# lukehollis/three-mlagents

Hardware: NVIDIA B200
Metric: env_steps_per_sec (higher is better)
Workload: dtype f32+f64

## Files before the change

### profiles/rollout_ab.py

```python
from __future__ import annotations

import argparse
import json
import os
import shutil
import statistics
import subprocess
import sys
import tempfile

import numpy as np

ROOT = os.path.dirname(os.path.dirname(os.path.abspath(__file__)))


def _run(cmd, cwd):
    r = subprocess.run(cmd, cwd=cwd, capture_output=True, text=True)
    if r.returncode != 0:
        raise RuntimeError(f"{' '.join(cmd)} in {cwd} failed ({r.returncode}):\n{r.stdout[-2000:]}\n{r.stderr[-4000:]}")
    return r.stdout


def _bench(tree, steps, dump=None):
    cmd = [sys.executable, "bench.py", "--quick", "--steps", str(steps)] + (["--dump-outputs", dump] if dump else [])
    return json.loads(_run(cmd, tree).strip().splitlines()[-1])


def main():
    ap = argparse.ArgumentParser()
    ap.add_argument("--parent", required=True, help="untracked export of the parent commit")
    ap.add_argument("--rounds", type=int, default=4)
    ap.add_argument("--steps", type=int, default=200)
    ap.add_argument("--out", default=os.path.join(ROOT, "profiles", "rollout_direct_obs_ab_1gpu.json"))
    args = ap.parse_args()
    trees = {"parent": os.path.abspath(args.parent), "new": ROOT}
    q = "name,power.limit,clocks.max.sm"
    card = _run(["nvidia-smi", f"--query-gpu={q}", "--format=csv,noheader", "-i", "0"], ROOT).strip()
    result = {"card": dict(zip(q.split(","), [c.strip() for c in card.split(",")])),
              "bench": f"bench.py --quick --steps {args.steps}", "rounds": args.rounds}
    for tree in trees.values():
        _run([sys.executable, os.path.join(tree, "three-mlagents_b200", "build.py")], tree)
    tmp = tempfile.mkdtemp(prefix="rollout_ab_")
    try:
        for name, tree in trees.items():
            _bench(tree, 50, dump=os.path.join(tmp, name))
        result["dump_equal"] = {f: bool(np.array_equal(np.load(os.path.join(tmp, "parent", f)), np.load(os.path.join(tmp, "new", f))))
                                for f in ("obs.npy", "actions.npy", "rewards.npy", "dones.npy")}
    finally:
        shutil.rmtree(tmp, ignore_errors=True)
    runs = {name: [] for name in trees}
    for _ in range(args.rounds):
        for name, tree in trees.items():
            runs[name].append(_bench(tree, args.steps)["ms_per_step"] * 1e3)
            print(name, f"{runs[name][-1]:.2f} us", file=sys.stderr, flush=True)
    base = statistics.median(runs["parent"])
    result["runs"] = {name: {"us_per_launch": us, "median_us": statistics.median(us),
                             "spread": (max(us) - min(us)) / statistics.median(us),
                             "gain_vs_parent": 1.0 - statistics.median(us) / base} for name, us in runs.items()}
    os.makedirs(os.path.dirname(os.path.abspath(args.out)), exist_ok=True)
    with open(args.out, "w") as f:
        json.dump(result, f, indent=1)
    print(json.dumps(result))


if __name__ == "__main__":
    main()
```

### three-mlagents_b200/csrc/env_kernels.cu

```cuda
#include <stdarg.h>
#include <stdlib.h>
#include <string.h>
#include <new>
#include <type_traits>
#if defined(__x86_64__)
#include <immintrin.h>
#endif
#include "envs.cuh"
#include "env_handle.cuh"

static int order_after_device_path(tmla_env *h) {
    if (!h->dev_dirty) return TMLA_OK;
    h->dev_dirty = false;
    cudaStreamCaptureStatus cap = cudaStreamCaptureStatusNone;
    if (cudaStreamIsCapturing(h->dev_stream, &cap) != cudaSuccess || cap != cudaStreamCaptureStatusNone ||
        cudaEventRecord(h->dev_evt, h->dev_stream) != cudaSuccess) {
        cudaGetLastError();
        TMLA_CUDA(cudaDeviceSynchronize());
        return TMLA_OK;
    }
    TMLA_CUDA(cudaStreamWaitEvent(h->own_stream, h->dev_evt, 0));
    return TMLA_OK;
}

struct EnvPtrs { void *buf[4]; };

static constexpr int kBlock = 128;

template <int D, int BLOCK, bool STREAMING>
__device__ __forceinline__ void block_store_obs(const float *s_obs, float *dst, int valid_envs) {
    const int total = valid_envs * D;
    if ((reinterpret_cast<uintptr_t>(dst) & 15u) == 0) {
        const int nvec = total >> 2;
        const float4 *s4 = reinterpret_cast<const float4 *>(s_obs);
        float4 *d4 = reinterpret_cast<float4 *>(dst);
        for (int v = threadIdx.x; v < nvec; v += BLOCK) {
            if (STREAMING) st_stream_f4(d4 + v, s4[v]);
            else d4[v] = s4[v];
        }
        for (int e = (nvec << 2) + threadIdx.x; e < total; e += BLOCK) dst[e] = s_obs[e];
    } else {
        for (int e = threadIdx.x; e < total; e += BLOCK) dst[e] = s_obs[e];
    }
}

template <int D>
__device__ __forceinline__ void thread_store_obs(const float *o, float *dst) {
#pragma unroll
    for (int j = 0; j < D; ++j) dst[j] = o[j];
}

template <class Task>
__global__ void __launch_bounds__(kBlock) reset_kernel(EnvPtrs p, int64_t n, uint64_t seed, uint64_t env_base,
                                                       uint64_t k, uint32_t tag, float *obs) {
    __shared__ __align__(16) float s_obs[kBlock * Task::D];
    const int64_t i0 = (int64_t)blockIdx.x * kBlock, i = i0 + threadIdx.x;
    if (i < n) {
        typename Task::State s;
        Task::reset(s, seed, env_base + (uint64_t)i, k, tag);
        Task::store(p.buf, i, s);
        float o[Task::D];
        Task::observe(s, o);
#pragma unroll
        for (int j = 0; j < Task::D; ++j) s_obs[threadIdx.x * Task::D + j] = o[j];
    }
    __syncthreads();
    if (obs) block_store_obs<Task::D, kBlock, false>(s_obs, obs + i0 * Task::D, (int)min((int64_t)kBlock, n - i0));
}

template <class Task>
__global__ void get_state_kernel(EnvPtrs p, int64_t n, typename Task::Wire *aos) {
    const int64_t i = (int64_t)blockIdx.x * blockDim.x + threadIdx.x;
    if (i < n) aos[i] = Task::to_wire(Task::load(p.buf, i));
}
template <class Task>
__global__ void set_state_kernel(EnvPtrs p, int64_t n, const typename Task::Wire *aos) {
    const int64_t i = (int64_t)blockIdx.x * blockDim.x + threadIdx.x;
    if (i < n) Task::store(p.buf, i, Task::from_wire(aos[i]));
}

template <class Task>
__global__ void __launch_bounds__(kBlock)
step_kernel(EnvPtrs p, int64_t n, uint64_t seed, uint64_t env_base, uint64_t step_index,
            const int32_t *__restrict__ actions, float *__restrict__ obs, float *__restrict__ reward,
            uint8_t *__restrict__ done, uint8_t *__restrict__ truncated, float *__restrict__ terminal_obs,
            float *__restrict__ ep_return, int32_t *__restrict__ ep_length, int32_t *n_done, int *err_flag,
            float *__restrict__ compact, int32_t *__restrict__ host_flags, int host_seq, int act_u8,
            const int32_t *ready, int32_t *dev_ready, int chunk_ctas, EnvPtrs shadow) {
    constexpr int D = Task::D;
    __shared__ __align__(16) float s_obs[kBlock * D];
    __shared__ __align__(16) float s_rew[kBlock];
    __shared__ __align__(16) uint8_t s_flag[2 * kBlock];
    const int64_t i0 = (int64_t)blockIdx.x * kBlock, i = i0 + threadIdx.x;
    if (ready) {
        __shared__ int s_go;
        if (threadIdx.x == 0) {
            const int c = blockIdx.x / chunk_ctas;
            const bool leader = blockIdx.x == (unsigned)(c * chunk_ctas);
            const volatile int32_t *f = leader ? ready + c : dev_ready + c;
            unsigned long long t0, t1;
            asm volatile("mov.u64 %0, %%globaltimer;" : "=l"(t0));
            int v;
            while ((v = *f) != host_seq && v != ~host_seq) {
                asm volatile("mov.u64 %0, %%globaltimer;" : "=l"(t1));
                if (t1 - t0 > 2000000000ull) { v = ~host_seq; break; }
                if (leader) __nanosleep(100);
            }
            if (leader) { __threadfence_system(); *(volatile int32_t *)(dev_ready + c) = v; }
            __threadfence_system();
            s_go = v == host_seq;
        }
        __syncthreads();
        if (!s_go) return;
    }
    const bool wide = (n - i0 >= kBlock) && (((reinterpret_cast<uintptr_t>(reward + i0) | reinterpret_cast<uintptr_t>(done + i0) |
                                               reinterpret_cast<uintptr_t>(truncated + i0)) & 15u) == 0);
    if (i < n) {
        const typename Task::Consts cst = Task::load_consts();
        typename Task::State s = Task::load(p.buf, i);
        if (shadow.buf[0]) Task::store(shadow.buf, i, s);
        int a = act_u8 ? (int)reinterpret_cast<const uint8_t *>(actions)[i] : actions[i];
        if ((unsigned)a >= (unsigned)Task::A) { *err_flag = 1; a = min(max(a, 0), Task::A - 1); }
        float r; bool term, trunc;
        Task::step(cst, s, a, r, term, trunc);
        s.ep_ret = __fadd_rn(s.ep_ret, r);
        const bool d = term || trunc;
        if (wide) {
            s_rew[threadIdx.x] = r;
            s_flag[threadIdx.x] = d ? 1 : 0;
            s_flag[kBlock + threadIdx.x] = (trunc && !term) ? 1 : 0;
        } else {
            reward[i] = r;
            done[i] = d ? 1 : 0;
            truncated[i] = (trunc && !term) ? 1 : 0;
        }
        float o[D];
        Task::observe(s, o);
        if (d) {
            if (terminal_obs) thread_store_obs<D>(o, terminal_obs + i * D);
            if (ep_return) ep_return[i] = s.ep_ret;
            if (ep_length) ep_length[i] = s.steps;
            int slot = 0;
            if (n_done) slot = atomicAdd(n_done, 1);
            if (compact) {
                constexpr int RW = (3 + D + 3) & ~3;
                float rec[RW];
                rec[0] = __int_as_float((int)i); rec[1] = s.ep_ret; rec[2] = __int_as_float(s.steps);
#pragma unroll
                for (int j = 0; j < D; ++j) rec[3 + j] = o[j];
#pragma unroll
                for (int j = 3 + D; j < RW; ++j) rec[j] = 0.0f;
                float4 *dst = reinterpret_cast<float4 *>(compact + (int64_t)slot * RW);
#pragma unroll
                for (int q = 0; q < RW / 4; ++q) dst[q] = make_float4(rec[4 * q], rec[4 * q + 1], rec[4 * q + 2], rec[4 * q + 3]);
            }
            Task::reset(s, seed, env_base + (uint64_t)i, step_index + 1, TMLA_TAG_RESET);
            Task::observe(s, o);
        }
        Task::store(p.buf, i, s);
#pragma unroll
        for (int j = 0; j < D; ++j) s_obs[threadIdx.x * D + j] = o[j];
    }
    __syncthreads();
    block_store_obs<D, kBlock, false>(s_obs, obs + i0 * D, (int)min((int64_t)kBlock, n - i0));
    if (wide) {
        const int t = threadIdx.x;
        if (t < kBlock / 4) reinterpret_cast<float4 *>(reward + i0)[t] = reinterpret_cast<const float4 *>(s_rew)[t];
        else if (t < kBlock / 4 + kBlock / 16) reinterpret_cast<uint4 *>(done + i0)[t - kBlock / 4] = reinterpret_cast<const uint4 *>(s_flag)[t - kBlock / 4];
        else if (t < kBlock / 4 + kBlock / 8) reinterpret_cast<uint4 *>(truncated + i0)[t - kBlock / 4 - kBlock / 16] = reinterpret_cast<const uint4 *>(s_flag + kBlock)[t - kBlock / 4 - kBlock / 16];
    }
    if (host_flags) {
        __syncthreads();
        if (threadIdx.x == 0) {
            __threadfence_system();
            if (atomicAdd(n_done + 2, 1) == (int)gridDim.x - 1) {
                __threadfence();
                host_flags[0] = *(volatile int32_t *)n_done;
                host_flags[1] = *(volatile int32_t *)(n_done + 1);
                n_done[0] = 0; n_done[1] = 0; n_done[2] = 0;
                __threadfence_system();
                *(volatile int32_t *)(host_flags + 2) = host_seq;
            }
        }
    }
}

static constexpr int kRollBlock = 32;

template <int D>
__device__ __forceinline__ void stage_obs(float *stage, const float *o) {
    if (D % 2 == 0) {
        float2 *s2 = reinterpret_cast<float2 *>(stage + threadIdx.x * D);
#pragma unroll
        for (int j = 0; j < D / 2; ++j) s2[j] = make_float2(o[2 * j], o[2 * j + 1]);
    } else {
#pragma unroll
        for (int j = 0; j < D; ++j) stage[threadIdx.x * D + j] = o[j];
    }
}

template <class Task>
__global__ void __launch_bounds__(kRollBlock)
rollout_random_kernel(EnvPtrs p, int64_t n, uint64_t seed, uint64_t env_base, uint64_t step0, int T,
                      float *__restrict__ obs_buf, int32_t *__restrict__ act_buf, float *__restrict__ rew_buf,
                      uint8_t *__restrict__ done_buf) {
    constexpr int D = Task::D, BLOCK = kRollBlock;
    constexpr bool STAGED = (D != 4);
    constexpr int NVEC = BLOCK * D / 4;
    __shared__ __align__(16) float s_obs[STAGED ? 2 * BLOCK * D : 4];
    const int64_t i0 = (int64_t)blockIdx.x * BLOCK, i = i0 + threadIdx.x;
    const bool active = i < n;
    const int valid = (int)min((int64_t)BLOCK, n - i0);
    const uint64_t env_id = env_base + (uint64_t)i;
    const int64_t row_floats = n * D;
    const bool vec_ok = obs_buf && valid == BLOCK && ((reinterpret_cast<uintptr_t>(obs_buf + i0 * D) & 15u) == 0) &&
                        ((row_floats & 3) == 0);
    const typename Task::Consts cst = Task::load_consts();
    typename Task::State s;
    TmlaActionStream as;
    if (active) {
        s = Task::load(p.buf, i);
        as.seek(seed, env_id, step0, Task::A);
    }
    float *orow = obs_buf ? obs_buf + i0 * D : nullptr;
    int64_t off = i;
    for (int t = 0; t < T; ++t) {
        const uint64_t k = step0 + (uint64_t)t;
        float *stage = STAGED ? s_obs + (t & 1) * BLOCK * D : s_obs;
        if (active) {
            float o[D];
            Task::observe(s, o);
            if (STAGED) stage_obs<D>(stage, o);
            else if (obs_buf) {
                float *dst = obs_buf + off * 4;
                if ((reinterpret_cast<uintptr_t>(obs_buf) & 15u) == 0) st_stream_f4(reinterpret_cast<float4 *>(dst), make_float4(o[0], o[1], o[2], o[3]));
                else { dst[0] = o[0]; dst[1] = o[1]; dst[2] = o[2]; dst[3] = o[3]; }
            }
            const int a = as.next(seed, env_id, step0, (uint32_t)t, Task::A);
            float r; bool term, trunc;
            Task::step(cst, s, a, r, term, trunc);
            s.ep_ret = __fadd_rn(s.ep_ret, r);
            const bool d = term || trunc;
            if (act_buf) __stcs(act_buf + off, a);
            if (rew_buf) __stcs(rew_buf + off, r);
            if (done_buf) __stcs(done_buf + off, (uint8_t)(d ? 1 : 0));
            if (d) Task::reset(s, seed, env_id, k + 1, TMLA_TAG_RESET);
        }
        if (STAGED) {
            __syncthreads();
            if (vec_ok) {
                const float4 *s4 = reinterpret_cast<const float4 *>(stage);
                float4 *d4 = reinterpret_cast<float4 *>(orow);
#pragma unroll
                for (int v = 0; v < (NVEC + BLOCK - 1) / BLOCK; ++v) {
                    const int e = v * BLOCK + threadIdx.x;
                    if ((v + 1) * BLOCK <= NVEC || e < NVEC) st_stream_f4(d4 + e, s4[e]);
                }
            } else if (obs_buf) {
                block_store_obs<D, BLOCK, true>(stage, orow, valid);
            }
            if (orow) orow += row_floats;
        }
        off += n;
    }
    if (active) Task::store(p.buf, i, s);
}

#ifndef TMLA_SPARE_EVERY
#define TMLA_SPARE_EVERY 64
#endif
static constexpr int kSpareEvery = TMLA_SPARE_EVERY;
#ifndef TMLA_ROLLOUT_UNROLL
#define TMLA_ROLLOUT_UNROLL 2
#endif
static constexpr int kRollUnroll = TMLA_ROLLOUT_UNROLL;
static_assert((kSpareEvery & (kSpareEvery - 1)) == 0, "power of two");
template <class Task>
__global__ void __launch_bounds__(kRollBlock)
rollout_fast_kernel(EnvPtrs p, uint32_t n, uint64_t seed, uint64_t env_base, uint64_t step0, int T,
                    float4 *__restrict__ obs4, int32_t *__restrict__ act_buf, float *__restrict__ rew_buf,
                    uint8_t *__restrict__ done_buf) {
    constexpr int D = Task::D, BLOCK = kRollBlock, NVEC = BLOCK * D / 4;
    constexpr bool DIRECT = (D == 6);
    constexpr bool STAGED = (D != 4) && !DIRECT;
    static_assert((BLOCK * D) % 4 == 0, "block rows must be whole float4s");
    __shared__ __align__(16) float s_stage[STAGED ? 2 * BLOCK * D : 4];
    const uint32_t tid = threadIdx.x, i = blockIdx.x * BLOCK + tid;
    const uint64_t env_id = env_base + (uint64_t)i;
    const typename Task::Consts cst = Task::load_consts();
    typename Task::State s = Task::load(p.buf, i);
    TmlaActionStream as;
    as.seek(seed, env_id, step0, Task::A);
    uint32_t off = i;
    uint32_t voff = blockIdx.x * NVEC + tid;
    const uint32_t rowvec = n / 4 * D;
    uint32_t sb = 0;
    [[maybe_unused]] typename Task::Spare sp;
    [[maybe_unused]] bool have_spare = false;
#pragma unroll kRollUnroll
    for (int t = 0; t < T; ++t) {
        if constexpr (Task::HAS_SPARE) {
            if ((t & (kSpareEvery - 1)) == 0 && !have_spare) {
                sp = Task::draw(seed, env_id, Task::next_episode(s), TMLA_TAG_RESET);
                have_spare = true;
            }
        }
        float o[D];
        Task::observe(s, o);
        if constexpr (STAGED) {
            if constexpr (D % 2 == 0) {
                float2 *s2 = reinterpret_cast<float2 *>(s_stage + sb + tid * D);
#pragma unroll
                for (int j = 0; j < D / 2; ++j) s2[j] = make_float2(o[2 * j], o[2 * j + 1]);
            } else {
#pragma unroll
                for (int j = 0; j < D; ++j) s_stage[sb + tid * D + j] = o[j];
            }
        } else if constexpr (DIRECT) {
            float2 *d2 = reinterpret_cast<float2 *>(reinterpret_cast<float *>(obs4) + (size_t)off * D);
#pragma unroll
            for (int j = 0; j < D / 2; ++j) __stcs(d2 + j, make_float2(o[2 * j], o[2 * j + 1]));
        } else {
            st_stream_f4(obs4 + off, make_float4(o[0], o[1], o[2], o[3]));
        }
        const int a = as.next(seed, env_id, step0, (uint32_t)t, Task::A);
        float r; bool term, trunc;
        Task::step(cst, s, a, r, term, trunc);
        s.ep_ret = __fadd_rn(s.ep_ret, r);
        const bool d = term || trunc;
        __stcs(act_buf + off, a);
        __stcs(rew_buf + off, r);
        __stcs(done_buf + off, (uint8_t)(d ? 1 : 0));
        if (d) {
            if constexpr (Task::HAS_SPARE) {
                const uint32_t e = Task::next_episode(s);
                if (!have_spare) sp = Task::draw(seed, env_id, e, TMLA_TAG_RESET);
                Task::begin_episode(s, sp, e);
                have_spare = false;
            } else {
                Task::reset(s, seed, env_id, step0 + (uint64_t)t + 1, TMLA_TAG_RESET);
            }
        }
        if constexpr (STAGED) {
            if constexpr (BLOCK == 32) __syncwarp(); else __syncthreads();
            const float4 *s4 = reinterpret_cast<const float4 *>(s_stage + sb);
#pragma unroll
            for (int v = 0; v < (NVEC + BLOCK - 1) / BLOCK; ++v) {
                const int e = v * BLOCK + tid;
                if ((v + 1) * BLOCK <= NVEC || e < NVEC) st_stream_f4(obs4 + voff + v * BLOCK, s4[e]);
            }
            sb ^= BLOCK * D;
            voff += rowvec;
        }
        off += n;
    }
    Task::store(p.buf, i, s);
}

template <int A>
__device__ __forceinline__ void categorical(const float *l, bool deterministic, float u, int &action, float &logp) {
    float m = l[0];
#pragma unroll
    for (int j = 1; j < A; ++j) m = fmaxf(m, l[j]);
    float e[A], sum = 0.0f;
#pragma unroll
    for (int j = 0; j < A; ++j) { e[j] = expf(l[j] - m); sum += e[j]; }
    int a = 0;
    if (deterministic) {
#pragma unroll
        for (int j = 1; j < A; ++j) if (l[j] > l[a]) a = j;
    } else {
        const float target = u * sum;
        float c = 0.0f;
        a = A - 1;
        bool found = false;
#pragma unroll
        for (int j = 0; j < A; ++j) {
            c += e[j];
            if (!found && target < c) { a = j; found = true; }
        }
    }
    action = a;
    logp = (l[a] - m) - logf(sum);
}

template <class Task>
__global__ void __launch_bounds__(kBlock)
step_policy_kernel(EnvPtrs p, int64_t n, uint64_t seed, uint64_t env_base, uint64_t step_index,
                   const uint64_t *__restrict__ step_base, const float *__restrict__ logits, int deterministic,
                   int64_t row_index, float *__restrict__ obs_next, int32_t *__restrict__ act, float *__restrict__ logp_out,
                   float *__restrict__ rew, uint8_t *__restrict__ done, int32_t *trunc_count,
                   int32_t *__restrict__ trunc_index, float *__restrict__ trunc_obs, int32_t trunc_capacity,
                   float *ep_stats, float2 *__restrict__ ep_log, int32_t ep_log_cap, int32_t *ep_log_count) {
    constexpr int D = Task::D, A = Task::A;
    __shared__ __align__(16) float s_obs[kBlock * D];
    __shared__ float s_ep[3];
    const int64_t i0 = (int64_t)blockIdx.x * kBlock, i = i0 + threadIdx.x;
    const uint64_t k = step_base ? (*step_base + (uint64_t)row_index) : step_index;
    const unsigned lane = threadIdx.x & 31u, lanes_below = (1u << lane) - 1u;
    if (threadIdx.x < 3) s_ep[threadIdx.x] = 0.0f;
    __syncthreads();
    const bool live = i < n;
    const uint64_t env_id = env_base + (uint64_t)i;
    typename Task::State s;
    float o[D];
    bool d = false, trunc_only = false;
    float ep_r = 0.0f, ep_l = 0.0f;
    if (live) {
        const typename Task::Consts cst = Task::load_consts();
        s = Task::load(p.buf, i);
        float l[A];
#pragma unroll
        for (int j = 0; j < A; ++j) l[j] = logits[i * A + j];
        float u = 0.0f;
        if (!deterministic) u = tmla_u24(tmla_stream_block(seed, env_id, k, TMLA_TAG_SAMPLE, 0).x);
        int a; float lp;
        categorical<A>(l, deterministic != 0, u, a, lp);
        float r; bool term, trunc;
        Task::step(cst, s, a, r, term, trunc);
        s.ep_ret = __fadd_rn(s.ep_ret, r);
        d = term || trunc;
        trunc_only = trunc && !term;
        if (act) act[i] = a;
        if (logp_out) logp_out[i] = lp;
        rew[i] = r;
        done[i] = d ? 1 : 0;
        Task::observe(s, o);
        if (d) { ep_r = s.ep_ret; ep_l = (float)s.steps; }
    }
    if (trunc_count) {
        const unsigned m = __ballot_sync(0xffffffffu, trunc_only);
        if (m) {
            const int leader = __ffs(m) - 1;
            int base = 0;
            if ((int)lane == leader) base = atomicAdd(trunc_count, __popc(m));
            base = __shfl_sync(0xffffffffu, base, leader);
            if (trunc_only) {
                const int slot = base + __popc(m & lanes_below);
                if (slot < trunc_capacity) {
                    trunc_index[slot] = (int32_t)(row_index * n + i);
                    thread_store_obs<D>(o, trunc_obs + (int64_t)slot * D);
                }
            }
        }
    }
    const unsigned dm = __ballot_sync(0xffffffffu, d);
    if (dm) {
        if (ep_stats) {
            float wr = ep_r, wl = ep_l;
#pragma unroll
            for (int sh = 16; sh > 0; sh >>= 1) { wr += __shfl_xor_sync(0xffffffffu, wr, sh); wl += __shfl_xor_sync(0xffffffffu, wl, sh); }
            if (lane == 0) { atomicAdd(s_ep + 0, wr); atomicAdd(s_ep + 1, wl); atomicAdd(s_ep + 2, (float)__popc(dm)); }
        }
        if (ep_log) {
            const int leader = __ffs(dm) - 1;
            int base = 0;
            if ((int)lane == leader) base = atomicAdd(ep_log_count, __popc(dm));
            base = __shfl_sync(0xffffffffu, base, leader);
            if (d) {
                const int slot = base + __popc(dm & lanes_below);
                if (slot < ep_log_cap) ep_log[slot] = make_float2(ep_r, ep_l);
            }
        }
    }
    if (live) {
        if (d) {
            Task::reset(s, seed, env_id, k + 1, TMLA_TAG_RESET);
            Task::observe(s, o);
        }
        Task::store(p.buf, i, s);
#pragma unroll
        for (int j = 0; j < D; ++j) s_obs[threadIdx.x * D + j] = o[j];
    }
    __syncthreads();
    if (ep_stats && threadIdx.x == 0 && s_ep[2] > 0.0f) {
        atomicAdd(ep_stats + 0, s_ep[0]);
        atomicAdd(ep_stats + 1, s_ep[1]);
        atomicAdd(ep_stats + 2, s_ep[2]);
    }
    block_store_obs<D, kBlock, false>(s_obs, obs_next + i0 * D, (int)min((int64_t)kBlock, n - i0));
}

__global__ void counter_add_kernel(uint64_t *c, uint64_t n) { *c += n; }

__global__ void selftest_arith_kernel(unsigned long long *out) {
    const uint32_t tid = blockIdx.x * blockDim.x + threadIdx.x, nth = gridDim.x * blockDim.x;
    unsigned long long bad3 = 0;
    for (uint32_t bits = tid; bits < 0x41000000u; bits += nth) {
        const float x = __uint_as_float(bits);
        bad3 += (__float_as_uint(div3_rn(x)) != __float_as_uint(__fdiv_rn(x, 3.0f)));
    }
    if (bad3) atomicAdd(out + 0, bad3);
    if (tid < 11) {
        const float k = (float)((int)tid - 5);
        if (__float_as_uint(div5_rn(k)) != __float_as_uint(__fdiv_rn(k, 5.0f))) atomicAdd(out + 1, 1ull);
    }
    unsigned long long worst = 0;
    for (uint32_t j = tid; j < (1u << 22); j += nth) {
        const double x = kB3.max_tilt * (2.0 * ((double)j + 0.5) / 4194304.0 - 1.0);
        const long long a = __double_as_longlong(sin_small(x)), b = __double_as_longlong(sin(x));
        const unsigned long long d = (unsigned long long)(a > b ? a - b : b - a);
        worst = d > worst ? d : worst;
    }
    atomicMax(out + 2, worst);
}

#define TASK_SWITCH(task, CALL)                                   \
    switch (task) {                                               \
        case TMLA_BASIC: { using TaskT = BasicTask; CALL; } break;        \
        case TMLA_BALL3D: { using TaskT = Ball3DTask; CALL; } break;      \
        case TMLA_GRIDWORLD: { using TaskT = GridWorldTask; CALL; } break; \
        case TMLA_PUSH: { using TaskT = PushTask; CALL; } break;          \
        case TMLA_WALLJUMP: { using TaskT = WallJumpTask; CALL; } break;  \
        case TMLA_BRICKBREAK: { using TaskT = BrickBreakTask; CALL; } break; \
        case TMLA_BICYCLE: { using TaskT = BicycleTask; CALL; } break;       \
        case TMLA_GLIDER: { using TaskT = GliderTask; CALL; } break;         \
        default: tmla_set_error("unknown task %d", task); return TMLA_EINVAL; \
    }

static EnvPtrs ptrs_of(const tmla_env *h) {
    EnvPtrs p;
    for (int b = 0; b < 4; ++b) p.buf[b] = h->buf[b];
    return p;
}
static inline unsigned grid_for(int64_t n) { return (unsigned)ceil_div64(n, kBlock); }

static const int kObsDim[TMLA_NUM_TASKS] = {BasicTask::D, Ball3DTask::D, GridWorldTask::D, PushTask::D, WallJumpTask::D, BrickBreakTask::D, BicycleTask::D, GliderTask::D};
static const int kNumActions[TMLA_NUM_TASKS] = {BasicTask::A, Ball3DTask::A, GridWorldTask::A, PushTask::A, WallJumpTask::A, BrickBreakTask::A, BicycleTask::A, GliderTask::A};
static const int kMaxSteps[TMLA_NUM_TASKS] = {BasicTask::MAX_STEPS, Ball3DTask::MAX_STEPS, GridWorldTask::MAX_STEPS, PushTask::MAX_STEPS,
                                              WallJumpTask::MAX_STEPS, BrickBreakTask::MAX_STEPS, BicycleTask::MAX_STEPS, GliderTask::MAX_STEPS};
static const int kStateSize[TMLA_NUM_TASKS] = {(int)sizeof(tmla_basic_state), (int)sizeof(tmla_ball3d_state), (int)sizeof(tmla_gridworld_state),
                                               (int)sizeof(tmla_push_state), (int)sizeof(tmla_walljump_state), (int)sizeof(tmla_brickbreak_state),
                                               (int)sizeof(tmla_bicycle_state), (int)sizeof(tmla_glider_state)};

static inline int record_words(int D) { return (3 + D + 3) & ~3; }
struct StageLayout { size_t act, obs, rew, done, trunc, flags, crec, tobs, ret, len, end; };
static StageLayout stage_layout(int64_t n, int D) {
    auto up = [](size_t x) { return (x + 15) & ~(size_t)15; };
    StageLayout L;
    L.act = 0;
    L.obs = up(L.act + 4 * n);
    L.rew = L.obs + 4 * n * D;
    L.done = L.rew + 4 * n;
    L.trunc = L.done + n;
    L.flags = up(L.trunc + n);
    L.crec = L.flags + 16;
    L.tobs = up(L.crec + 4 * n * record_words(D));
    L.ret = L.tobs + 4 * n * D;
    L.len = L.ret + 4 * n;
    L.end = L.len + 4 * n;
    return L;
}


#if defined(__x86_64__)
__attribute__((target("avx2"))) static int64_t stage_actions32_avx2(const int32_t *src, uint8_t *dst, int64_t n, uint64_t *ored, uint32_t *mx) {
    __m256i acc = _mm256_setzero_si256(), vmx = _mm256_setzero_si256();
    const __m256i perm = _mm256_setr_epi32(0, 4, 1, 5, 2, 6, 3, 7);
    int64_t i = 0;
    for (; i + 32 <= n; i += 32) {
        const __m256i a = _mm256_loadu_si256((const __m256i *)(src + i)), b = _mm256_loadu_si256((const __m256i *)(src + i + 8));
        const __m256i c = _mm256_loadu_si256((const __m256i *)(src + i + 16)), d = _mm256_loadu_si256((const __m256i *)(src + i + 24));
        acc = _mm256_or_si256(acc, _mm256_or_si256(_mm256_or_si256(a, b), _mm256_or_si256(c, d)));
        __m256i p = _mm256_packus_epi16(_mm256_packs_epi32(a, b), _mm256_packs_epi32(c, d));
        p = _mm256_permutevar8x32_epi32(p, perm);
        vmx = _mm256_max_epu8(vmx, p);
        _mm256_storeu_si256((__m256i *)(dst + i), p);
    }
    uint64_t t[4]; uint8_t m8[32];
    _mm256_storeu_si256((__m256i *)t, acc); _mm256_storeu_si256((__m256i *)m8, vmx);
    const uint64_t o = t[0] | t[1] | t[2] | t[3];
    *ored |= (o | (o >> 32)) & 0xFFFFFFFFull;
    for (int k = 0; k < 32; ++k) *mx = m8[k] > *mx ? m8[k] : *mx;
    return i;
}
__attribute__((target("avx2"))) static int64_t stage_actions64_avx2(const int64_t *src, uint8_t *dst, int64_t n, uint64_t *ored, uint32_t *mx) {
    __m256i acc = _mm256_setzero_si256(), vmx = _mm256_setzero_si256();
    const __m256i lo = _mm256_setr_epi32(0, 2, 4, 6, 0, 2, 4, 6), perm = _mm256_setr_epi32(0, 4, 1, 5, 2, 6, 3, 7);
    int64_t i = 0;
    for (; i + 32 <= n; i += 32) {
        __m256i w[4];
        for (int k = 0; k < 4; ++k) {
            const __m256i x = _mm256_loadu_si256((const __m256i *)(src + i + 8 * k)), y = _mm256_loadu_si256((const __m256i *)(src + i + 8 * k + 4));
            acc = _mm256_or_si256(acc, _mm256_or_si256(x, y));
            const __m256i xl = _mm256_permutevar8x32_epi32(x, lo), yl = _mm256_permutevar8x32_epi32(y, lo);
            w[k] = _mm256_inserti128_si256(xl, _mm256_castsi256_si128(yl), 1);
        }
        __m256i p = _mm256_packus_epi16(_mm256_packs_epi32(w[0], w[1]), _mm256_packs_epi32(w[2], w[3]));
        p = _mm256_permutevar8x32_epi32(p, perm);
        vmx = _mm256_max_epu8(vmx, p);
        _mm256_storeu_si256((__m256i *)(dst + i), p);
    }
    uint64_t t[4]; uint8_t m8[32];
    _mm256_storeu_si256((__m256i *)t, acc); _mm256_storeu_si256((__m256i *)m8, vmx);
    const uint64_t o = t[0] | t[1] | t[2] | t[3];
    *ored |= (o & ~7ull) ? 0xFFFFFFFFull : (o & 7ull);
    for (int k = 0; k < 32; ++k) *mx = m8[k] > *mx ? m8[k] : *mx;
    return i;
}
#endif

extern "C" {

int tmla_task_from_name(const char *name) {
    if (!name) { tmla_set_error("task name is NULL"); return TMLA_EINVAL; }
    if (!strcmp(name, "basic")) return TMLA_BASIC;
    if (!strcmp(name, "ball3d")) return TMLA_BALL3D;
    if (!strcmp(name, "gridworld")) return TMLA_GRIDWORLD;
    if (!strcmp(name, "push")) return TMLA_PUSH;
    if (!strcmp(name, "walljump")) return TMLA_WALLJUMP;
    if (!strcmp(name, "brickbreak")) return TMLA_BRICKBREAK;
    if (!strcmp(name, "bicycle")) return TMLA_BICYCLE;
    if (!strcmp(name, "glider")) return TMLA_GLIDER;
    tmla_set_error("no CUDA backend for task '%s' (have: basic, ball3d, gridworld, push, walljump, brickbreak, bicycle, glider)", name);
    return TMLA_EINVAL;
}
#define TASK_META(fn, table)                                                                   \
    int fn(int task) {                                                                         \
        if (task < 0 || task >= TMLA_NUM_TASKS) { tmla_set_error(#fn ": unknown task %d", task); return TMLA_EINVAL; } \
        return table[task];                                                                    \
    }
TASK_META(tmla_task_obs_dim, kObsDim)
TASK_META(tmla_task_num_actions, kNumActions)
TASK_META(tmla_task_max_steps, kMaxSteps)
TASK_META(tmla_task_state_size, kStateSize)

int tmla_create(int task, int64_t n_envs, uint64_t seed, uint64_t env_id_base, int device, tmla_env **out) {
    TMLA_REQUIRE(out != nullptr, "out is NULL");
    TMLA_REQUIRE(task >= 0 && task < TMLA_NUM_TASKS, "unknown task");
    TMLA_REQUIRE(n_envs > 0 && n_envs < (int64_t)1 << 31, "n_envs must be in (0, 2^31)");
    int ndev = 0;
    TMLA_CUDA(cudaGetDeviceCount(&ndev));
    TMLA_REQUIRE(device >= 0 && device < ndev, "no such CUDA device (this library has no CPU path)");
    DeviceGuard guard(device);
    tmla_env *h = new (std::nothrow) tmla_env();
    if (!h) { tmla_set_error("out of host memory"); return TMLA_ENOMEM; }
    memset(h, 0, sizeof(*h));
    h->task = task; h->n = n_envs; h->seed = seed; h->env_id_base = env_id_base; h->device = device;
    h->rec_hint = 256;
    int nbuf = 0;
    size_t pb[4] = {0, 0, 0, 0};
    TASK_SWITCH(task, nbuf = TaskT::NBUF; for (int b = 0; b < nbuf; ++b) pb[b] = TaskT::plane_bytes(b));
    for (int b = 0; b < nbuf; ++b) {
        cudaError_t e = cudaMalloc(&h->buf[b], pb[b] * (size_t)n_envs);
        if (e != cudaSuccess) { tmla_set_error("cudaMalloc(state plane %d): %s", b, cudaGetErrorString(e)); tmla_destroy(h); return TMLA_ENOMEM; }
    }
    const int D = kObsDim[task];
    h->stage_bytes = stage_layout(n_envs, D).end + 64;
    if (cudaMalloc(&h->d_stage, h->stage_bytes) != cudaSuccess || cudaMallocHost(&h->h_stage, h->stage_bytes) != cudaSuccess ||
        cudaMalloc((void **)&h->err_flag, sizeof(int)) != cudaSuccess || cudaMalloc((void **)&h->d_ndone, sizeof(int32_t)) != cudaSuccess ||
        cudaStreamCreateWithFlags(&h->own_stream, cudaStreamNonBlocking) != cudaSuccess ||
        cudaEventCreateWithFlags(&h->dev_evt, cudaEventDisableTiming) != cudaSuccess) {
        tmla_set_error("allocating staging buffers: %s", cudaGetErrorString(cudaGetLastError()));
        tmla_destroy(h);
        return TMLA_ENOMEM;
    }
    TMLA_CUDA(cudaMemset(h->err_flag, 0, sizeof(int)));
// ... 477 lines not shown
```

### three-mlagents_b200/csrc/philox.cuh

```cuda
#pragma once
#include <stdint.h>

#define TMLA_TAG_RESET 0u
#define TMLA_TAG_ACTION 1u
#define TMLA_TAG_SAMPLE 2u
#define TMLA_TAG_PERM 3u
#define TMLA_TAG_RESET_ALL 4u

__host__ __device__ __forceinline__ uint4 philox4x32_10(uint4 c, uint2 k) {
#pragma unroll
    for (int r = 0; r < 10; ++r) {
        uint64_t p0 = (uint64_t)0xD2511F53u * c.x;
        uint64_t p1 = (uint64_t)0xCD9E8D57u * c.z;
        uint4 n;
        n.x = (uint32_t)(p1 >> 32) ^ c.y ^ k.x;
        n.y = (uint32_t)p1;
        n.z = (uint32_t)(p0 >> 32) ^ c.w ^ k.y;
        n.w = (uint32_t)p0;
        c = n;
        k.x += 0x9E3779B9u;
        k.y += 0xBB67AE85u;
    }
    return c;
}

__host__ __device__ __forceinline__ uint4 tmla_stream_block(uint64_t seed, uint64_t env_id, uint64_t k,
                                                            uint32_t tag, uint32_t block) {
    uint4 c;
    c.x = (uint32_t)env_id;
    c.y = (uint32_t)(env_id >> 32);
    c.z = (uint32_t)k;
    c.w = ((uint32_t)(k >> 32) << 8) | (block << 4) | tag;
    return philox4x32_10(c, make_uint2((uint32_t)seed, (uint32_t)(seed >> 32)));
}

__host__ __device__ __forceinline__ int tmla_bounded(uint32_t x, uint32_t n) {
    return (int)(((uint64_t)x * n) >> 32);
}
__host__ __device__ __forceinline__ double tmla_u53(uint32_t a, uint32_t b) {
    return ((double)(a >> 5) * 67108864.0 + (double)(b >> 6)) * (1.0 / 9007199254740992.0);
}
__host__ __device__ __forceinline__ float tmla_u24(uint32_t a) { return (float)(a >> 8) * (1.0f / 16777216.0f); }

struct TmlaActionStream {
    uint4 blk;
    uint32_t frac;
    __device__ __forceinline__ static uint32_t word_of(const uint4 &b, uint32_t w) {
        return w == 0 ? b.x : (w == 1 ? b.y : (w == 2 ? b.z : b.w));
    }
    __device__ __forceinline__ void seek(uint64_t seed, uint64_t env_id, uint64_t k, uint32_t n_actions) {
        blk = tmla_stream_block(seed, env_id, k >> 4, TMLA_TAG_ACTION, 0);
        frac = word_of(blk, (uint32_t)(k & 15u) >> 2);
        for (uint32_t d = 0; d < (uint32_t)(k & 3u); ++d) frac = (uint32_t)((uint64_t)frac * n_actions);
    }
    __device__ __forceinline__ int next(uint64_t seed, uint64_t env_id, uint64_t step0, uint32_t t, uint32_t n_actions) {
        const uint32_t j = ((uint32_t)step0 + t) & 15u;
        if ((j & 3u) == 0) {
            if (j == 0 && t != 0) blk = tmla_stream_block(seed, env_id, (step0 + t) >> 4, TMLA_TAG_ACTION, 0);
            frac = word_of(blk, j >> 2);
        }
        const uint64_t p = (uint64_t)frac * n_actions;
        frac = (uint32_t)p;
        return (int)(p >> 32);
    }
};
```

Before: 144.7 billion.

## Restructure rollout loop into 16-step action blocks with precomputed packed action digits

The rollout kernel now iterates over 16-step blocks. For each block it computes one Philox call and packs all 16 actions as 4-bit digits in a 64-bit word, so the per-step branchy action-stream state machine goes away and full blocks are unrolled. Per-step offsets become pointer increments, and the rare reset draw moves to a noinline helper to keep the hot loop small. It also adds SASS and per-task timing profiling scripts. The cost is extra code for partial blocks and a limit of 16 actions.

Measured after the change: 151.4 billion, median of 6. 4.6% higher.

```diff
diff --git a/profiles/rollout_ab.py b/profiles/rollout_ab.py
--- a/profiles/rollout_ab.py
+++ b/profiles/rollout_ab.py
@@ -26,12 +26,45 @@
     return json.loads(_run(cmd, tree).strip().splitlines()[-1])
 
 
+_TASK_TIMER = """
+import sys, torch
+sys.path.insert(0, '.')
+from three_mlagents_b200.vec_env import CudaVecEnv
+task, n, T, K = sys.argv[1], 65536, 128, int(sys.argv[2])
+env = CudaVecEnv(task, n, seed=1)
+obs = torch.empty((T, n, env.obs_dim), device='cuda')
+act = torch.empty((T, n), dtype=torch.int32, device='cuda')
+rew = torch.empty((T, n), device='cuda')
+done = torch.empty((T, n), dtype=torch.uint8, device='cuda')
+for _ in range(50):
+    env.rollout_random(T, obs, act, rew, done)
+e0, e1 = torch.cuda.Event(enable_timing=True), torch.cuda.Event(enable_timing=True)
+e0.record()
+for _ in range(K):
+    env.rollout_random(T, obs, act, rew, done)
+e1.record()
+torch.cuda.synchronize()
+print(e0.elapsed_time(e1) / K * 1e3)
+"""
+
+
+def _time_task(tree, task, steps):
+    return float(_run([sys.executable, "-c", _TASK_TIMER, task, str(steps)], tree).strip().splitlines()[-1])
+
+
+def _summary(runs, base_name="parent"):
+    base = statistics.median(runs[base_name])
+    return {name: {"us_per_launch": us, "median_us": statistics.median(us), "spread": (max(us) - min(us)) / statistics.median(us),
+                   "gain_vs_parent": 1.0 - statistics.median(us) / base} for name, us in runs.items()}
+
+
 def main():
     ap = argparse.ArgumentParser()
     ap.add_argument("--parent", required=True, help="untracked export of the parent commit")
     ap.add_argument("--rounds", type=int, default=4)
     ap.add_argument("--steps", type=int, default=200)
-    ap.add_argument("--out", default=os.path.join(ROOT, "profiles", "rollout_direct_obs_ab_1gpu.json"))
+    ap.add_argument("--tasks", default="gridworld,push", help="tasks also timed through env.rollout_random ('' for none)")
+    ap.add_argument("--out", default=os.path.join(ROOT, "profiles", "rollout_blocks_ab_1gpu.json"))
     args = ap.parse_args()
     trees = {"parent": os.path.abspath(args.parent), "new": ROOT}
     q = "name,power.limit,clocks.max.sm"
@@ -48,15 +81,19 @@
                                 for f in ("obs.npy", "actions.npy", "rewards.npy", "dones.npy")}
     finally:
         shutil.rmtree(tmp, ignore_errors=True)
+    tasks = [t for t in args.tasks.split(",") if t]
     runs = {name: [] for name in trees}
+    task_runs = {task: {name: [] for name in trees} for task in tasks}
     for _ in range(args.rounds):
         for name, tree in trees.items():
             runs[name].append(_bench(tree, args.steps)["ms_per_step"] * 1e3)
             print(name, f"{runs[name][-1]:.2f} us", file=sys.stderr, flush=True)
-    base = statistics.median(runs["parent"])
-    result["runs"] = {name: {"us_per_launch": us, "median_us": statistics.median(us),
-                             "spread": (max(us) - min(us)) / statistics.median(us),
-                             "gain_vs_parent": 1.0 - statistics.median(us) / base} for name, us in runs.items()}
+            for task in tasks:
+                task_runs[task][name].append(_time_task(tree, task, args.steps))
+                print(name, task, f"{task_runs[task][name][-1]:.2f} us", file=sys.stderr, flush=True)
+    result["runs"] = _summary(runs)
+    if tasks:
+        result["rollout_random_65536x128"] = {task: _summary(r) for task, r in task_runs.items()}
     os.makedirs(os.path.dirname(os.path.abspath(args.out)), exist_ok=True)
     with open(args.out, "w") as f:
         json.dump(result, f, indent=1)
diff --git a/profiles/rollout_sass.py b/profiles/rollout_sass.py
--- /dev/null
+++ b/profiles/rollout_sass.py
@@ -0,0 +1,108 @@
+from __future__ import annotations
+
+import argparse
+import os
+import re
+import subprocess
+import sys
+import tempfile
+
+ROOT = os.path.dirname(os.path.dirname(os.path.abspath(__file__)))
+FLAGS = ["-gencode", "arch=compute_100a,code=sm_100a", "-lineinfo", "-O3", "-std=c++17", "--expt-relaxed-constexpr"]
+INS = re.compile(r"^\s+/\*([0-9a-f]{4,})\*/\s+(.*?)\s*;")
+
+
+def _compile(tree, tmp):
+    csrc = os.path.join(tree, "three-mlagents_b200", "csrc")
+    cubin = os.path.join(tmp, "env_kernels.cubin")
+    nvcc = os.path.join(os.environ.get("CUDA_HOME", "/usr/local/cuda"), "bin", "nvcc")
+    r = subprocess.run([nvcc, *FLAGS, "-I", os.path.join(tree, "include"), "-Xptxas", "-v", "-cubin", "-o", cubin,
+                        os.path.join(csrc, "env_kernels.cu")], capture_output=True, text=True)
+    if r.returncode != 0:
+        raise SystemExit(r.stdout + r.stderr)
+    return cubin, r.stdout + r.stderr
+
+
+def _ptxas(log, mangled):
+    lines = log.splitlines()
+    for n, line in enumerate(lines):
+        if f"'{mangled}'" in line and "Compiling entry" in line:
+            text = " ".join(lines[n + 1:n + 4])
+            num = lambda pat: int(re.search(pat, text).group(1))
+            return {"registers": num(r"Used (\d+) registers"), "stack_bytes": num(r"(\d+) bytes stack frame"),
+                    "spill_store_bytes": num(r"(\d+) bytes spill stores"), "spill_load_bytes": num(r"(\d+) bytes spill loads")}
+    raise SystemExit(f"{mangled}: no ptxas report")
+
+
+def _sass(cubin, mangled):
+    out = subprocess.run(["cuobjdump", "-sass", "-fun", mangled, cubin], capture_output=True, text=True, check=True).stdout
+    return [(int(m.group(1), 16), m.group(2)) for m in map(INS.match, out.splitlines()) if m]
+
+
+def _branch(ins):
+    m = re.match(r"(@!?U?P\w+\s+)?BRA(\.U)?\s+(!?U?P\w+,\s*)?(0x[0-9a-f]+)", ins)
+    if not m:
+        return None
+    return int(m.group(4), 16), bool(m.group(1) or m.group(3))
+
+
+def _loops(code):
+    loops = []
+    for addr, ins in code:
+        b = _branch(ins)
+        if b and b[0] <= addr:
+            loops.append((b[0], addr))
+    return [(h, e) for h, e in loops if not any(h <= h2 and e2 <= e and (h2, e2) != (h, e) for h2, e2 in loops)]
+
+
+def _shortest(code, head, end):
+    body = [(a, ins) for a, ins in code if head <= a <= end]
+    index = {a: n for n, (a, _) in enumerate(body)}
+    inf = (1 << 30, 0, 0)
+    best = [inf] * (len(body) + 1)
+    best[0] = (0, 0, 0)
+    for n, (a, ins) in enumerate(body):
+        if best[n] == inf:
+            continue
+        c, br, st = best[n]
+        here = (c + 1, br + (_branch(ins) is not None), st + ("STG" in ins and ".U8" in ins))
+        if a == end:
+            best[len(body)] = min(best[len(body)], here)
+            continue
+        b = _branch(ins)
+        nxt = []
+        if b is None or b[1]:
+            if not re.match(r"(EXIT|RET)", ins):
+                nxt.append(n + 1)
+        if b and head < b[0] <= end and b[0] in index:
+            nxt.append(index[b[0]])
+        for m in nxt:
+            best[m] = min(best[m], here)
+    return best[len(body)]
+
+
+def main():
+    ap = argparse.ArgumentParser()
+    ap.add_argument("--tree", default=ROOT, help="repository tree whose env_kernels.cu is compiled")
+    ap.add_argument("--tasks", default="Ball3D,GridWorld,Push")
+    args = ap.parse_args()
+    with tempfile.TemporaryDirectory(prefix="rollout_sass_") as tmp:
+        cubin, log = _compile(os.path.abspath(args.tree), tmp)
+        for task in args.tasks.split(","):
+            name = f"{task}Task"
+            mangled = f"_Z19rollout_fast_kernelI{len(name)}{name}Ev7EnvPtrsjmmmiP6float4PiPfPh"
+            res = _ptxas(log, mangled)
+            code = _sass(cubin, mangled)
+            print(f"rollout_fast_kernel<{name}>: {res['registers']} registers, stack {res['stack_bytes']} B, "
+                  f"spills {res['spill_store_bytes']} B stored / {res['spill_load_bytes']} B loaded, {len(code) * 16} B of code")
+            for head, end in _loops(code):
+                ins, br, steps = _shortest(code, head, end)
+                if not steps:
+                    continue
+                per = f", per step {ins / steps:.1f} instructions and {br / steps:.1f} branches"
+                print(f"    loop 0x{head:x}-0x{end:x}: {end + 16 - head} B, shortest path {ins} instructions, "
+                      f"{br} branches, {steps} steps{per}")
+
+
+if __name__ == "__main__":
+    sys.exit(main())
diff --git a/three-mlagents_b200/csrc/env_kernels.cu b/three-mlagents_b200/csrc/env_kernels.cu
--- a/three-mlagents_b200/csrc/env_kernels.cu
+++ b/three-mlagents_b200/csrc/env_kernels.cu
@@ -274,13 +274,21 @@
 #define TMLA_ROLLOUT_UNROLL 2
 #endif
 static constexpr int kRollUnroll = TMLA_ROLLOUT_UNROLL;
-static_assert((kSpareEvery & (kSpareEvery - 1)) == 0, "power of two");
+static_assert(kSpareEvery % 16 == 0 && ((kSpareEvery / 16) & (kSpareEvery / 16 - 1)) == 0, "a power-of-two number of action blocks");
+static_assert(16 % kRollUnroll == 0, "the unrolled step loop covers whole action blocks");
+
+template <class Task>
+__device__ __noinline__ typename Task::Spare draw_spare(uint64_t seed, uint64_t env_id, uint32_t episode) {
+    return Task::draw(seed, env_id, episode, TMLA_TAG_RESET);
+}
+
 template <class Task>
 __global__ void __launch_bounds__(kRollBlock)
 rollout_fast_kernel(EnvPtrs p, uint32_t n, uint64_t seed, uint64_t env_base, uint64_t step0, int T,
                     float4 *__restrict__ obs4, int32_t *__restrict__ act_buf, float *__restrict__ rew_buf,
                     uint8_t *__restrict__ done_buf) {
     constexpr int D = Task::D, BLOCK = kRollBlock, NVEC = BLOCK * D / 4;
+    static_assert(Task::A <= 16, "actions are packed as 4-bit digits");
     constexpr bool DIRECT = (D == 6);
     constexpr bool STAGED = (D != 4) && !DIRECT;
     static_assert((BLOCK * D) % 4 == 0, "block rows must be whole float4s");
@@ -289,56 +297,50 @@
     const uint64_t env_id = env_base + (uint64_t)i;
     const typename Task::Consts cst = Task::load_consts();
     typename Task::State s = Task::load(p.buf, i);
-    TmlaActionStream as;
-    as.seek(seed, env_id, step0, Task::A);
-    uint32_t off = i;
-    uint32_t voff = blockIdx.x * NVEC + tid;
-    const uint32_t rowvec = n / 4 * D;
+    float *orow = reinterpret_cast<float *>(obs4) + (size_t)i * D;
+    float4 *vrow = obs4 + blockIdx.x * NVEC + tid;
+    int32_t *arow = act_buf + i;
+    float *rrow = rew_buf + i;
+    uint8_t *drow = done_buf + i;
+    const uint32_t rowfloats = n * D;
     uint32_t sb = 0;
     [[maybe_unused]] typename Task::Spare sp;
     [[maybe_unused]] bool have_spare = false;
-#pragma unroll kRollUnroll
-    for (int t = 0; t < T; ++t) {
-        if constexpr (Task::HAS_SPARE) {
-            if ((t & (kSpareEvery - 1)) == 0 && !have_spare) {
-                sp = Task::draw(seed, env_id, Task::next_episode(s), TMLA_TAG_RESET);
-                have_spare = true;
-            }
-        }
+    auto step = [&](uint64_t digits, uint32_t j, uint64_t kb) {
         float o[D];
         Task::observe(s, o);
         if constexpr (STAGED) {
             if constexpr (D % 2 == 0) {
                 float2 *s2 = reinterpret_cast<float2 *>(s_stage + sb + tid * D);
 #pragma unroll
-                for (int j = 0; j < D / 2; ++j) s2[j] = make_float2(o[2 * j], o[2 * j + 1]);
+                for (int q = 0; q < D / 2; ++q) s2[q] = make_float2(o[2 * q], o[2 * q + 1]);
             } else {
 #pragma unroll
-                for (int j = 0; j < D; ++j) s_stage[sb + tid * D + j] = o[j];
+                for (int q = 0; q < D; ++q) s_stage[sb + tid * D + q] = o[q];
             }
         } else if constexpr (DIRECT) {
-            float2 *d2 = reinterpret_cast<float2 *>(reinterpret_cast<float *>(obs4) + (size_t)off * D);
-#pragma unroll
-            for (int j = 0; j < D / 2; ++j) __stcs(d2 + j, make_float2(o[2 * j], o[2 * j + 1]));
+            float2 *d2 = reinterpret_cast<float2 *>(orow);
+#pragma unroll
+            for (int q = 0; q < D / 2; ++q) __stcs(d2 + q, make_float2(o[2 * q], o[2 * q + 1]));
         } else {
-            st_stream_f4(obs4 + off, make_float4(o[0], o[1], o[2], o[3]));
-        }
-        const int a = as.next(seed, env_id, step0, (uint32_t)t, Task::A);
+            st_stream_f4(reinterpret_cast<float4 *>(orow), make_float4(o[0], o[1], o[2], o[3]));
+        }
+        const int a = (int)((uint32_t)(digits >> (4 * j)) & 15u);
         float r; bool term, trunc;
         Task::step(cst, s, a, r, term, trunc);
         s.ep_ret = __fadd_rn(s.ep_ret, r);
         const bool d = term || trunc;
-        __stcs(act_buf + off, a);
-        __stcs(rew_buf + off, r);
-        __stcs(done_buf + off, (uint8_t)(d ? 1 : 0));
+        __stcs(arow, a);
+        __stcs(rrow, r);
+        __stcs(drow, (uint8_t)(d ? 1 : 0));
         if (d) {
             if constexpr (Task::HAS_SPARE) {
                 const uint32_t e = Task::next_episode(s);
-                if (!have_spare) sp = Task::draw(seed, env_id, e, TMLA_TAG_RESET);
+                if (!have_spare) sp = draw_spare<Task>(seed, env_id, e);
                 Task::begin_episode(s, sp, e);
                 have_spare = false;
             } else {
-                Task::reset(s, seed, env_id, step0 + (uint64_t)t + 1, TMLA_TAG_RESET);
+                Task::reset(s, seed, env_id, kb + j + 1, TMLA_TAG_RESET);
             }
         }
         if constexpr (STAGED) {
@@ -347,12 +349,36 @@
 #pragma unroll
             for (int v = 0; v < (NVEC + BLOCK - 1) / BLOCK; ++v) {
                 const int e = v * BLOCK + tid;
-                if ((v + 1) * BLOCK <= NVEC || e < NVEC) st_stream_f4(obs4 + voff + v * BLOCK, s4[e]);
+                if ((v + 1) * BLOCK <= NVEC || e < NVEC) st_stream_f4(vrow + v * BLOCK, s4[e]);
             }
             sb ^= BLOCK * D;
-            voff += rowvec;
-        }
-        off += n;
+            vrow += rowfloats / 4;
+        } else {
+            orow += rowfloats;
+        }
+        arow += n; rrow += n; drow += n;
+    };
+    uint64_t kb = step0 & ~(uint64_t)15;
+    uint32_t j = (uint32_t)step0 & 15u;
+    uint32_t left = (uint32_t)T;
+    for (uint32_t nb = 0; left != 0; ++nb, kb += 16, j = 0) {
+        const uint64_t digits = TmlaActionStream::block_digits(seed, env_id, kb >> 4, Task::A);
+        if constexpr (Task::HAS_SPARE) {
+            if ((nb & (kSpareEvery / 16 - 1)) == 0 && !have_spare) {
+                sp = Task::draw(seed, env_id, Task::next_episode(s), TMLA_TAG_RESET);
+                have_spare = true;
+            }
+        }
+        if (j == 0 && left >= 16) {
+#pragma unroll kRollUnroll
+            for (uint32_t q = 0; q < 16; ++q) step(digits, q, kb);
+            left -= 16;
+        } else {
+            const uint32_t je = min(16u, j + left);
+            left -= je - j;
+#pragma unroll 1
+            for (; j < je; ++j) step(digits, j, kb);
+        }
     }
     Task::store(p.buf, i, s);
 }
diff --git a/three-mlagents_b200/csrc/philox.cuh b/three-mlagents_b200/csrc/philox.cuh
--- a/three-mlagents_b200/csrc/philox.cuh
+++ b/three-mlagents_b200/csrc/philox.cuh
@@ -63,4 +63,20 @@
         frac = (uint32_t)p;
         return (int)(p >> 32);
     }
+    __device__ __forceinline__ static uint64_t block_digits(uint64_t seed, uint64_t env_id, uint64_t blk, uint32_t n_actions) {
+        const uint4 b = tmla_stream_block(seed, env_id, blk, TMLA_TAG_ACTION, 0);
+        const uint32_t w[4] = {b.x, b.y, b.z, b.w};
+        uint32_t half[2] = {0u, 0u};
+#pragma unroll
+        for (int q = 0; q < 4; ++q) {
+            uint32_t frac = w[q];
+#pragma unroll
+            for (int d = 0; d < 4; ++d) {
+                const uint64_t p = (uint64_t)frac * n_actions;
+                frac = (uint32_t)p;
+                half[q >> 1] |= (uint32_t)(p >> 32) << (4 * (4 * (q & 1) + d));
+            }
+        }
+        return ((uint64_t)half[1] << 32) | half[0];
+    }
 };
```
